# banyancomputer/hot-proofs-blake3-circom

Hardware: AMD Instinct MI355X
Metric: BLAKE3-compression witnesses/sec (higher is better)
Workload: dtype u32

## Files before the change

### hot-proofs-blake3-circom_amd/__init__.py

```python
import ctypes
import os
import re

import numpy as np

from . import workloads


def __getattr__(name):
    if name in ("sharding", "chain", "bao"):
        import importlib
        return importlib.import_module(__name__ + "." + name)
    raise AttributeError(name)

PKG_DIR = os.path.dirname(os.path.abspath(__file__))
LIB_PATH = os.environ.get("B3WIT_LIB") or os.path.join(PKG_DIR, "libb3wit.so")

CIRCUITS = ("compression", "nova_bn254", "nova_vesta", "nova_bn254_o1")
CIRCUIT_ID = {c: i for i, c in enumerate(CIRCUITS)}

B3W_OK = 0
PLACEMENT_NAMES = {0: "plain", 1: "mixed", 2: "interleaved"}
B3W_E_ASSERT_FAILED = 4
B3W_E_BAD_ARGUMENT = 100
# ... 65 lines not shown
        "b3w_bodies_stats": (i32, [vp, vp]),
        "b3w_bodies_search_stats": (i32, [vp, ctypes.POINTER(ctypes.c_double)]),
        "b3w_bodies_search_limit": (None, [ctypes.c_double]),
        "b3w_bodies_search_breakdown": (i32, [vp, ctypes.POINTER(ctypes.c_double)]),
        "b3w_bodies_store_rate": (i32, [vp, vp, u32, u64, i32, u32, vp, ctypes.POINTER(ctypes.c_double)]),
        "b3w_batch_placement": (i32, [vp]),
        "b3w_chain_num_chunks": (u64, [u64]),
        "b3w_chain_num_leaf_steps": (u64, [u64]),
        "b3w_chain_path_len": (u32, [u64, u64]),
        "b3w_chain_num_parent_steps": (u64, [u64, u64, u64]),
        "b3w_chain_parent_row": (u64, [u64, u64]),
        "b3w_chain_path_provable": (i32, [u64, u64]),
        "b3w_chain_plan_leaves_device": (i32, [vp, vp, u64, u64, u32, vp, vp, vp]),
        "b3w_chain_tree_device": (i32, [vp, vp, u64, vp, vp]),
        "b3w_chain_plan_parents_device": (i32, [vp, vp, u64, u64, u64, u32, vp, vp]),
        "b3w_commit_key_create": (i32, [vp, i32, u32, vp, ctypes.POINTER(vp)]),
        "b3w_commit_key_create_ex": (i32, [vp, i32, u32, vp, u32, ctypes.POINTER(vp)]),
        "b3w_commit_key_create_folded": (i32, [vp, i32, u32, vp, vp, u32, ctypes.POINTER(vp)]),
        "b3w_slot_widths": (i32, [vp, vp]),
        "b3w_commit_key_window": (u32, [vp]),
        "b3w_commit_key_destroy": (None, [vp]),
        "b3w_commit_key_count": (i32, [vp, i32]),
        "b3w_commit_key_counts": (i32, [vp, ctypes.POINTER(u64)]),
        "b3w_commit_records_device": (i32, [vp, vp, vp, u32, vp, vp, vp, vp]),
        "b3w_commit_records": (i32, [vp, vp, vp, u32, vp, vp, vp]),
        "b3w_chain_commit_only": (i32, [vp, vp, vp]),
        "b3w_chain_commit_from_records": (i32, [vp, vp, vp]),
        "b3w_chain_commit_overlap": (i32, [vp, i32]),
        "b3w_chain_violations_device": (vp, [vp]),
        "b3w_chain_commitments": (i32, [vp, vp, vp]),
        "b3w_chain_check_constraints": (i32, [vp, vp]),
        "b3w_chain_violations": (i32, [vp, vp, vp]),
        "b3w_batch_commit_device": (i32, [vp, vp, vp, u32, u64, vp, vp, vp]),
        "b3w_batch_commit": (i32, [vp, vp, vp, vp]),
        "b3w_commit_consumer": (None, [vp, vp, u64, u64, u32, vp]),
        "b3w_comm_unique_id": (i32, [vp]),
        "b3w_comm_create": (i32, [vp, vp, i32, i32, ctypes.POINTER(vp)]),
        "b3w_comm_create_host": (i32, [vp, ctypes.c_char_p, i32, i32, ctypes.POINTER(vp)]),
        "b3w_comm_create_external": (i32, [vp, i32, i32, vp, vp, ctypes.POINTER(vp)]),
        "b3w_comm_rank": (i32, [vp]),
        "b3w_comm_size": (i32, [vp]),
        "b3w_comm_destroy": (None, [vp]),
        "b3w_comm_allgather": (i32, [vp, vp, vp, u64, vp]),
        "b3w_batch_allgather_public": (i32, [vp, vp, vp]),
        "b3w_chain_create": (i32, [vp, u64, u64, u32, u32, u32, i32, ctypes.POINTER(vp)]),
        "b3w_chain_destroy": (None, [vp]),
# ... 40 lines not shown
        "b3w_bao_stream_outboard_begin": (i32, [vp, u64, u32, vp, vp, vp, u64, ctypes.POINTER(vp)]),
        "b3w_bao_stream_verify_begin": (i32, [vp, u64, u32, vp, vp, vp, vp, vp, vp, u64, vp, ctypes.POINTER(vp)]),
        "b3w_bao_stream_push": (i32, [vp, u64, vp, u64, vp]),
        "b3w_bao_stream_finish": (i32, [vp, vp]),
        "b3w_bao_stream_free": (None, [vp]),
        "b3w_sample_plan_arena_device": (i32, [vp, vp, u64, vp, vp, u32, u32, vp, vp, vp, vp, u32, vp, vp, vp]),
        "b3w_bao_slice_arena_device": (i32, [vp, vp, u64, vp, vp, u32, u32, vp, vp, vp, u32, vp, vp]),
    }
    for name, (res, args) in sig.items():
        fn = getattr(L, name)
        fn.restype, fn.argtypes = res, args
    _lib = L
    return L


EXPORTED_SYMBOLS = ("b3w_abi_version", "b3w_identify_wasm", "b3w_create", "b3w_destroy", "b3w_info",
                    "b3w_input_signal_size", "b3w_calc_witness", "b3w_write_wtns_header", "b3w_last_error",
                    "b3w_batch_run_device", "b3w_public_words", "b3w_batch_alloc", "b3w_batch_free",
                    "b3w_batch_run", "b3w_batch_outputs", "b3w_batch_fetch", "b3w_batch_device_ptr",
                    "b3w_batch_time_device", "b3w_batch_verify_device", "b3w_batch_verify",
                    "b3w_r1cs_create", "b3w_r1cs_info", "b3w_r1cs_is_tiled", "b3w_r1cs_destroy", "b3w_r1cs_check_device", "b3w_batch_r1cs_check", "b3w_r1cs_consumer", "b3w_batch_write_wtns", "b3w_batch_write_wtns_ex", "b3w_batch_autotune_device", "b3w_bodies_alloc", "b3w_bodies_free", "b3w_bodies_trim", "b3w_ctx_trim", "b3w_bodies_configure", "b3w_bodies_stats", "b3w_bodies_search_stats", "b3w_bodies_search_limit", "b3w_bodies_search_breakdown", "b3w_bodies_store_rate", "b3w_batch_placement", "b3w_chain_num_chunks", "b3w_chain_num_leaf_steps", "b3w_chain_path_len",
                    "b3w_chain_num_parent_steps", "b3w_chain_parent_row", "b3w_chain_path_provable",
                    "b3w_chain_plan_leaves_device", "b3w_chain_tree_device", "b3w_chain_plan_parents_device",
                    "b3w_commit_key_create", "b3w_commit_key_create_ex", "b3w_commit_key_create_folded", "b3w_slot_widths", "b3w_commit_key_window", "b3w_commit_key_destroy", "b3w_commit_key_count", "b3w_commit_key_counts", "b3w_commit_records_device", "b3w_commit_records", "b3w_chain_commit_only", "b3w_chain_commit_from_records", "b3w_chain_commit_overlap", "b3w_chain_violations_device", "b3w_chain_commitments", "b3w_chain_check_constraints", "b3w_chain_violations", "b3w_batch_commit_device", "b3w_batch_commit", "b3w_commit_consumer",
                    "b3w_comm_unique_id", "b3w_comm_create", "b3w_comm_create_host", "b3w_comm_create_external", "b3w_comm_rank", "b3w_comm_size", "b3w_comm_destroy", "b3w_comm_allgather", "b3w_batch_allgather_public",
                    "b3w_chain_create", "b3w_chain_destroy", "b3w_chain_run_leaves", "b3w_chain_run_parents", "b3w_chain_shard", "b3w_chain_run_parents_sharded", "b3w_chain_allgather_hout", "b3w_chain_allgather_hout_host", "b3w_chain_exchange_ms", "b3w_chain_info",
                    "b3w_chain_outputs", "b3w_chain_records", "b3w_chain_public", "b3w_chain_status", "b3w_chain_local_cvs", "b3w_chain_root",
                    "b3w_bao_outboard_size", "b3w_bao_outboard_device", "b3w_bao_path_nodes", "b3w_bao_slice", "b3w_sample_rows",
                    "b3w_sample_plan_device", "b3w_bao_batch_layout", "b3w_bao_batch_scratch_bytes", "b3w_bao_outboard_batch_device",
                    "b3w_sample_rows_batch", "b3w_sample_plan_batch_device", "b3w_bao_group_outboard_size", "b3w_bao_group_batch_layout",
                    "b3w_bao_group_path_nodes", "b3w_bao_group_outboard_batch_device", "b3w_sample_plan_group_batch_device",
                    "b3w_bao_slice_size", "b3w_bao_slice_batch_layout", "b3w_bao_slice_decode", "b3w_bao_slice_batch_device",
                    "b3w_sample_plan_slices_device",
                    "b3w_bao_verify_layout", "b3w_bao_verify_scratch_bytes", "b3w_bao_verify_batch_device", "b3w_bao_verify",
                    "b3w_bao_stream_scratch_bytes", "b3w_bao_stream_outboard_begin", "b3w_bao_stream_verify_begin", "b3w_bao_stream_push",
                    "b3w_bao_stream_finish", "b3w_bao_stream_free",
                    "b3w_sample_plan_arena_device", "b3w_bao_slice_arena_device")


class graph_capture:

    def __init__(self, graph, stream=None, **kw):
        import torch
        self._inner = torch.cuda.graph(graph, stream=stream, **kw)
        self._gc_was_on = False

    def __enter__(self):
# ... 346 lines not shown
    def commit_records_device(self, d_records, n, d_points, d_status, d_public=0, stream=0):
        rc = lib().b3w_commit_records_device(self.ctx.handle, self.handle, d_records, n, d_points, d_public or None, d_status, stream or None)
        if rc != B3W_OK:
            raise B3WError(rc, f"b3w_commit_records_device: status {rc}: {self.ctx.last_error()}")

    def commit_records(self, records):
        recs = np.ascontiguousarray(records, dtype=np.uint32)
        n = recs.shape[0]
        pts = np.zeros((n, 64), dtype=np.uint8)
        pub = np.zeros((n, self.ctx.public_words), dtype=np.uint32)
        st = np.zeros(n, dtype=np.int32)
        rc = lib().b3w_commit_records(self.ctx.handle, self.handle, recs.ctypes.data, n, pts.ctypes.data, pub.ctypes.data, st.ctypes.data)
        if rc != B3W_OK:
            raise B3WError(rc, f"b3w_commit_records: status {rc}: {self.ctx.last_error()}")
        return pts, pub, st

    def count(self, on=True):
        lib().b3w_commit_key_count(self.handle, 1 if on else 0)

    def counts(self):
        out = (ctypes.c_uint64 * 2)()
        lib().b3w_commit_key_counts(self.handle, out)
        return int(out[0]), int(out[1])

    def close(self):
        if getattr(self, "handle", None):
            lib().b3w_commit_key_destroy(self.handle)
            self.handle = None

    def __del__(self):
        try:
            self.close()
        except Exception:
            pass


class ChainPlanner:

    def __init__(self, ctx):
        self.ctx = ctx

    def _chk(self, rc, what):
        if rc != B3W_OK:
            raise B3WError(rc, f"{what}: status {rc}: {self.ctx.last_error()}")

    def parent_rows(self, n_chunks, first_chunk=0, n_chunks_local=None):
# ... 218 lines not shown
```

### hot-proofs-blake3-circom_amd/csrc/b3w_commit.hip

```cpp
#include <hip/hip_runtime.h>
#include <stdint.h>
#include <stdlib.h>
#include "b3w_kernels.h"
#include "b3w_atoms.h"

namespace {

struct Fp { uint32_t l[8]; };
struct Jac { Fp X, Y, Z; };

__device__ __forceinline__ bool fp_is_zero(const Fp &a) {
  uint32_t o = 0;
#pragma unroll
  for (int i = 0; i < 8; ++i) o |= a.l[i];
  return o == 0;
}
__device__ __forceinline__ bool fp_eq(const Fp &a, const Fp &b) {
  uint32_t o = 0;
#pragma unroll
  for (int i = 0; i < 8; ++i) o |= a.l[i] ^ b.l[i];
  return o == 0;
}
__device__ __forceinline__ Fp fp_zero() { Fp r; for (int i = 0; i < 8; ++i) r.l[i] = 0; return r; }

// ... 539 lines not shown
#pragma unroll
  for (int i = 0; i < 8; ++i) r2.l[i] = C.r2[i];
  const Fp gx = fp_mul(load_fp(gens + (uint64_t)s * 16), r2, C), gy = fp_mul(load_fp(gens + (uint64_t)s * 16 + 8), r2, C);
  const uint32_t *sc = inverses + 8ull * mag;
  Jac R = jac_infinity();
#pragma unroll 1
  for (int b = 255; b >= 0; --b) {
    R = jac_dbl(R, C);
    if ((sc[b >> 5] >> (b & 31)) & 1u) R = jac_madd(R, gx, gy, C);
  }
  Fp x, y, c32;
  jac_to_affine(R, x, y, C);
#pragma unroll
  for (int k = 0; k < 8; ++k) c32.l[k] = C.one[k];
#pragma unroll 1
  for (int k = 0; k < 5; ++k) c32 = fp_dbl(c32, C);
  const Fp xo = fp_mul(x, c32, C);
  store_fp(o, xo);
  store_fp(o + 8, fp_mul(y, c32, C));
  store_fp(on, xo);
  store_fp(on + 8, fp_mul(fp_sub(fp_zero(), y, C), c32, C));
}

#define B3W_WINDOW_K 4
template <int W>
__global__ __launch_bounds__(64) void b3w_commit_window_kernel(const uint32_t *__restrict__ points, uint32_t nwin,
                                                               uint32_t *__restrict__ table, B3wCurve C, B3wCurve9 C9) {
  constexpr int K = B3W_WINDOW_K;
  constexpr uint32_t CHUNKS = (1u << W) / K;
  __shared__ uint32_t lds[5 * K * 9 * 64];
  const uint32_t tid = threadIdx.x;
  const uint64_t gid = (uint64_t)blockIdx.x * 64 + tid;
  if (gid >= (uint64_t)nwin * CHUNKS) return;
  const uint32_t win = (uint32_t)(gid / CHUNKS), g0 = (uint32_t)(gid % CHUNKS) * K;
  auto at = [&](int what, int e, int l) -> uint32_t & { return lds[((what * K + e) * 9 + l) * 64 + tid]; };
  auto point = [&](uint32_t b, bool negate, F9 &x, F9 &y) {
    const uint32_t *pt = points + (uint64_t)(win * W + b) * 16;
    Fp py = load_fp(pt + 8);
    if (negate) py = fp_sub(fp_zero(), py, C);
    x = to29(load_fp(pt)); y = to29(py);
  };
  J9 acc = j9_infinity();
  const uint32_t m0 = g0 ^ (g0 >> 1);
#pragma unroll 1
  for (uint32_t b = 0; b < (uint32_t)W; ++b) {
    if (!((m0 >> b) & 1)) continue;
    F9 x, y;
    point(b, false, x, y);
    j9_madd(acc, x, y, C9);
  }
#pragma unroll 1
  for (int e = 0; e < K; ++e) {
    if (e > 0) {
      const uint32_t g = g0 + e, m = g ^ (g >> 1), b = (uint32_t)__builtin_ctz(g);
      F9 x, y;
      point(b, !((m >> b) & 1), x, y);
      j9_madd(acc, x, y, C9);
    }
    const F9 A = acc.inf ? one29(C9) : mul29(acc.ZZ, acc.ZZZ, C9);
#pragma unroll
    for (int l = 0; l < 9; ++l) {
      at(0, e, l) = acc.X.l[l]; at(1, e, l) = acc.Y.l[l];
      at(2, e, l) = acc.inf ? 0u : acc.ZZ.l[l]; at(3, e, l) = acc.inf ? 0u : acc.ZZZ.l[l];
    }
    F9 c;
    if (e == 0) c = A;
    else {
#pragma unroll
      for (int l = 0; l < 9; ++l) c.l[l] = at(4, e - 1, l);
      c = mul29(c, A, C9);
    }
#pragma unroll
    for (int l = 0; l < 9; ++l) at(4, e, l) = c.l[l];
  }
  F9 inv;
#pragma unroll
  for (int l = 0; l < 9; ++l) inv.l[l] = at(4, K - 1, l);
  inv = inv29(inv, C.pm2, C9);
#pragma unroll 1
  for (int e = K - 1; e >= 0; --e) {
// ... 351 lines not shown
  D.sp4[8] -= 1u;
  uint32_t x[8];
  for (int i = 0; i < 8; ++i) x[i] = C.one[i];
  for (int k = 0; k < 5; ++k) u256_dbl_mod_h(x, C.p);
  for (int i = 0; i < 8; ++i) w[i] = x[i];
  w[8] = 0;
  u288_split29(w, D.one);
  D.inv = C.inv & M29;
  const uint64_t phi = ((uint64_t)C.p[7] << 32) | C.p[6];
  D.mu = (uint32_t)((((unsigned __int128)1) << 77) / ((unsigned __int128)phi + 1));
  for (uint32_t k = 3; k <= 5; ++k) D.kp0[k - 3] = (k * D.p[0]) & M29;
  return D;
}

}

extern "C" int b3w_launch_commit_setup(const uint32_t *d_gens, const uint32_t *d_first_v, const uint32_t *d_nbits, uint32_t nslots,
                                       uint32_t *d_points, const B3wCurve *curve, hipStream_t stream) {
  if (!nslots) return 0;
  hipLaunchKernelGGL(b3w_commit_setup_kernel, dim3(nslots), dim3(64), 0, stream, d_gens, d_first_v, d_nbits, nslots, d_points, *curve);
  return (int)hipGetLastError();
}

extern "C" int b3w_launch_commit_windows(const uint32_t *d_points, uint32_t nwin, uint32_t window, uint32_t *d_table, const B3wCurve *curve, hipStream_t stream) {
  if (!nwin) return 0;
  if (!B3W_COMMIT_WINDOW_OK(window)) return (int)hipErrorInvalidValue;
  const uint64_t total = (uint64_t)nwin * ((1u << window) / B3W_WINDOW_K);
  const dim3 grid((uint32_t)((total + 63) / 64));
  const B3wCurve9 c9 = make_curve9(*curve);
  if (window == B3W_COMMIT_WINDOW_XL)
    hipLaunchKernelGGL(b3w_commit_window_kernel<B3W_COMMIT_WINDOW_XL>, grid, dim3(64), 0, stream, d_points, nwin, d_table, *curve, c9);
  else if (window == B3W_COMMIT_WINDOW_LARGE)
    hipLaunchKernelGGL(b3w_commit_window_kernel<B3W_COMMIT_WINDOW_LARGE>, grid, dim3(64), 0, stream, d_points, nwin, d_table, *curve, c9);
  else
    hipLaunchKernelGGL(b3w_commit_window_kernel<B3W_COMMIT_WINDOW_SMALL>, grid, dim3(64), 0, stream, d_points, nwin, d_table, *curve, c9);
  return (int)hipGetLastError();
}

extern "C" int b3w_launch_commit(const uint8_t *d_bodies, uint32_t n, uint64_t pitch, uint32_t first_slot, uint32_t nslots,
                                 const uint32_t *d_slotdesc, const uint32_t *d_images , uint32_t img_row, const uint32_t *d_runs,
                                 uint32_t nruns, const uint32_t *d_table, uint32_t nwin, uint32_t window,
                                 uint32_t *d_sums , uint8_t *d_out, int32_t *d_status,
                                 const uint32_t *d_invtab, uint32_t inv_nk, const uint32_t *d_invmeta, const uint32_t *d_aux,
                                 unsigned long long *d_adds, const B3wCurve *curve, hipStream_t stream) {
  if (!n) return 0;
  if (!d_images && !(d_invtab && d_invmeta && d_aux)) { d_invtab = nullptr; d_invmeta = nullptr; }
// ... 55 lines not shown
```

### hot-proofs-blake3-circom_amd/csrc/b3w_commit_api.cpp

```cpp
#include "b3w_internal.h"


struct b3w_commit_key {
  b3w_ctx *ctx = nullptr;
  B3wCurve curve{};
  uint32_t first_slot = 0, nwin = 0, window = 0;
  uint32_t nslots = 0;
  uint32_t *d_slotdesc = nullptr;
  uint32_t *d_runs = nullptr; uint32_t nruns = 0;
  uint32_t *d_images = nullptr; uint32_t images_cap = 0;
  uint32_t *d_table = nullptr;
  uint32_t *d_invtab = nullptr; uint32_t inv_nk = 0;
  uint32_t *d_invmeta = nullptr;
  uint32_t *d_sums = nullptr;
  uint32_t sums_cap = 0;
  unsigned long long *d_counts = nullptr;
  uint64_t host_witnesses = 0;
  bool counting = false;
};

namespace {
bool u256_geq(const uint32_t a[8], const uint32_t b[8]) { for (int i = 7; i >= 0; --i) if (a[i] != b[i]) return a[i] > b[i]; return true; }
void u256_sub_host(uint32_t a[8], const uint32_t b[8]) {
  uint64_t br = 0;
  for (int i = 0; i < 8; i++) { const uint64_t t = (uint64_t)a[i] - b[i] - br; a[i] = (uint32_t)t; br = (t >> 63) & 1; }
}
void u256_double_mod(uint32_t a[8], const uint32_t p[8]) {
  uint32_t c = 0;
  for (int i = 0; i < 8; i++) { const uint32_t n = (a[i] << 1) | c; c = a[i] >> 31; a[i] = n; }
  if (c || u256_geq(a, p)) u256_sub_host(a, p);
}
B3wCurve make_curve(const uint64_t p64[4]) {
  B3wCurve C{};
  memcpy(C.p, p64, 32);
  uint32_t x[8] = {1, 0, 0, 0, 0, 0, 0, 0};
  for (int i = 0; i < 256; i++) u256_double_mod(x, C.p);
  memcpy(C.one, x, 32);
  for (int i = 0; i < 256; i++) u256_double_mod(x, C.p);
  memcpy(C.r2, x, 32);
  memcpy(C.pm2, C.p, 32);
  const uint32_t two[8] = {2, 0, 0, 0, 0, 0, 0, 0};
  u256_sub_host(C.pm2, two);
  uint32_t inv = C.p[0];
  for (int i = 0; i < 5; i++) inv *= 2u - C.p[0] * inv;
  C.inv = 0u - inv;
  return C;
}
const uint64_t Q_BN254[4] = {0x3c208c16d87cfd47ull, 0x97816a916871ca8dull, 0xb85045b68181585dull, 0x30644e72e131a029ull};
const uint64_t P_VESTA_BASE[4] = {0x992d30ed00000001ull, 0x224698fc094cf91bull, 0x0ull, 0x4000000000000000ull};
}

extern "C" {

int32_t b3w_commit_key_create(b3w_ctx *ctx, int32_t curve, uint32_t first_slot, const uint8_t *host_generators, b3w_commit_key **out) {
  return b3w_commit_key_create_ex(ctx, curve, first_slot, host_generators, 0, out);
}

uint32_t b3w_commit_key_window(const b3w_commit_key *key) { return key ? key->window : 0; }

int32_t b3w_commit_key_create_ex(b3w_ctx *ctx, int32_t curve, uint32_t first_slot, const uint8_t *host_generators, uint32_t window_bits,
                                 b3w_commit_key **out) {
  return b3w_commit_key_create_folded(ctx, curve, first_slot, host_generators, nullptr, window_bits, out);
}

int32_t b3w_slot_widths(b3w_ctx *ctx, uint16_t *out_bits) {
  if (!ctx || !out_bits) return B3W_E_BAD_ARGUMENT;
  std::vector<uint32_t> table;
  if (!b3w_int_build_slot_table(ctx->desc, table, ctx->last_error)) return B3W_E_BAD_ARGUMENT;
  for (uint32_t i = 0; i < ctx->desc.nwit; i++) {
// ... 131 lines not shown
  if (e == hipSuccess) e = hipMalloc((void **)&key->d_slotdesc, (size_t)nslots * 4);
  if (e == hipSuccess) e = hipMemcpy(key->d_slotdesc, desc.data(), (size_t)nslots * 4, hipMemcpyHostToDevice);
  if (e == hipSuccess) e = hipMalloc((void **)&key->d_table, (size_t)key->nwin * B3W_COMMIT_ENTRIES(window) * 64);
  if (e == hipSuccess) e = hipMalloc((void **)&d_points, (size_t)nv * 64);
  if (e == hipSuccess) e = hipMalloc((void **)&d_gens, (size_t)nslots * 64);
  if (e == hipSuccess) e = hipMalloc((void **)&d_first, (size_t)nslots * 4);
  if (e == hipSuccess) e = hipMalloc((void **)&d_nbits, (size_t)nslots * 4);
  if (e == hipSuccess) e = hipMemcpy(d_gens, host_generators, (size_t)nslots * 64, hipMemcpyHostToDevice);
  if (e == hipSuccess) e = hipMemcpy(d_first, first_v.data(), (size_t)nslots * 4, hipMemcpyHostToDevice);
  if (e == hipSuccess) e = hipMemcpy(d_nbits, nbits.data(), (size_t)nslots * 4, hipMemcpyHostToDevice);
  int rc = e == hipSuccess ? b3w_launch_commit_setup(d_gens, d_first, d_nbits, nslots, d_points, &key->curve, nullptr) : 0;
  for (uint32_t v = V0; v < nv && e == hipSuccess && rc == 0; v++)
    e = hipMemcpyAsync(d_points + (size_t)v * 16, d_points, 64, hipMemcpyDeviceToDevice, nullptr);
  if (e == hipSuccess && rc == 0) rc = b3w_launch_commit_windows(d_points, key->nwin, key->window, key->d_table, &key->curve, nullptr);
  if (e == hipSuccess && rc == 0 && with_invtab) {
    key->inv_nk = B3W_INV_TABLE_N - 1;
    e = hipMalloc((void **)&key->d_invmeta, invmeta.size() * 4);
    if (e == hipSuccess) e = hipMemcpy(key->d_invmeta, invmeta.data(), invmeta.size() * 4, hipMemcpyHostToDevice);
    if (e == hipSuccess) e = hipMalloc((void **)&key->d_invtab, (size_t)B3W_NOVA_ISZERO * 2 * key->inv_nk * 64);
    if (e == hipSuccess)
      rc = b3w_launch_commit_invtab(d_gens, key->d_invmeta, static_cast<const uint32_t *>(ctx->d_aux) + 16, B3W_NOVA_ISZERO, key->inv_nk, key->d_invtab, &key->curve,
                                    nullptr);
  }
  if (e == hipSuccess && rc == 0) e = hipDeviceSynchronize();
  if (d_gens) (void)hipFree(d_gens);
  if (d_first) (void)hipFree(d_first);
  if (d_nbits) (void)hipFree(d_nbits);
  if (d_points) (void)hipFree(d_points);
  if (e != hipSuccess || rc != 0) {
    b3w_commit_key_destroy(key);
    *herr = e != hipSuccess ? e : (hipError_t)rc;
    (void)hipGetLastError();
    return hip_fail(ctx, e != hipSuccess ? e : (hipError_t)rc, "commitment key set-up");
  }
  *out = key;
  return B3W_OK;
}

void b3w_commit_key_destroy(b3w_commit_key *key) {
  if (!key) return;
  B3wCaptureRelaxed relaxed;
  DeviceGuard guard(key->ctx->device);
  if (key->d_slotdesc) (void)hipFree(key->d_slotdesc);
  if (key->d_invmeta) (void)hipFree(key->d_invmeta);
  if (key->d_runs) (void)hipFree(key->d_runs);
  if (key->d_images) (void)hipFree(key->d_images);
  if (key->d_table) (void)hipFree(key->d_table);
  if (key->d_invtab) (void)hipFree(key->d_invtab);
  if (key->d_sums) (void)hipFree(key->d_sums);
  if (key->d_counts) (void)hipFree(key->d_counts);
  delete key;
}

int32_t b3w_commit_key_count(b3w_commit_key *key, int32_t on) {
  if (!key) return B3W_E_BAD_ARGUMENT;
  b3w_ctx *ctx = key->ctx;
  ON_DEVICE(ctx);
  HIP_TRY(ctx, hipDeviceSynchronize());
  if (on && !key->d_counts) HIP_TRY(ctx, hipMalloc((void **)&key->d_counts, 8));
  if (on) { HIP_TRY(ctx, hipMemset(key->d_counts, 0, 8)); key->host_witnesses = 0; }
  key->counting = on != 0;
  return B3W_OK;
}

int32_t b3w_commit_key_counts(const b3w_commit_key *key, uint64_t out[2]) {
  if (!key || !out) return B3W_E_BAD_ARGUMENT;
  b3w_ctx *ctx = key->ctx;
  out[0] = 0; out[1] = key->host_witnesses;
  if (!key->d_counts) return B3W_OK;
  ON_DEVICE(ctx);
  HIP_TRY(ctx, hipDeviceSynchronize());
  unsigned long long v = 0;
  HIP_TRY(ctx, hipMemcpy(&v, key->d_counts, 8, hipMemcpyDeviceToHost));
  out[0] = v;
  return B3W_OK;
}

int32_t b3w_batch_commit_device(b3w_ctx *ctx, const b3w_commit_key *key, const uint8_t *d_bodies, uint32_t n, uint64_t pitch,
                                uint8_t *d_points, int32_t *d_status, void *stream) {
  if (!ctx || !key || key->ctx != ctx || !d_bodies || !d_points) return B3W_E_BAD_ARGUMENT;
  const uint64_t body = 32ull * ctx->desc.nwit;
  if (pitch == 0) pitch = body;
  if (pitch < body || (pitch & 15) || (reinterpret_cast<uintptr_t>(d_bodies) & 15) || (reinterpret_cast<uintptr_t>(d_points) & 15)) {
    ctx->last_error = "pitch must be >= witness_size*32 and a multiple of 16, bodies and points 16-byte aligned";
// ... 40 lines not shown
    return B3W_E_BAD_ARGUMENT;
  }
  ON_DEVICE(ctx);
  b3w_commit_key *k = const_cast<b3w_commit_key *>(key);
  constexpr uint32_t CHUNK = 32768;
  const uint32_t want = std::min(n, CHUNK);
  if (k->images_cap < want || k->sums_cap < want) {
    HIP_TRY(ctx, hipStreamSynchronize((hipStream_t)stream));
    if (split) HIP_TRY(ctx, hipStreamSynchronize((hipStream_t)trace_stream));
    if (k->sums_cap < want) {
      if (k->d_sums) (void)hipFree(k->d_sums);
      k->d_sums = nullptr; k->sums_cap = 0;
      HIP_TRY(ctx, hipMalloc((void **)&k->d_sums, (size_t)want * B3W_COMMIT_SUM_WORDS * 4));
      k->sums_cap = want;
    }
    if (k->images_cap < want) {
      if (k->d_images) (void)hipFree(k->d_images);
      k->d_images = nullptr; k->images_cap = 0;
      HIP_TRY(ctx, hipMalloc((void **)&k->d_images, (size_t)want * ctx->desc.lds_words * 4));
      k->images_cap = want;
    }
  }
  const uint32_t cap = k->images_cap;
  const uint32_t rw = ctx->desc.nin, pw = ctx->desc.npub;
  for (uint32_t c0 = 0; c0 < n; c0 += cap) {
    const uint32_t cn = std::min(cap, n - c0);
    int lrc = b3w_launch_trace(ctx->desc.kind, d_records + (uint64_t)c0 * rw, cn, k->d_images, cap, ctx->d_table, ctx->desc.nwit,
                               d_public ? d_public + (uint64_t)c0 * pw : nullptr, d_status + c0, ctx->d_aux, (hipStream_t)(split ? trace_stream : stream));
    if (lrc == 0 && split) {
      hipError_t e = hipEventRecord(trace_done, (hipStream_t)trace_stream);
      if (e == hipSuccess) e = hipStreamWaitEvent((hipStream_t)stream, trace_done, 0);
      if (e != hipSuccess) return hip_fail(ctx, e, "TRACE event");
    }
    if (lrc == 0)
      lrc = b3w_launch_commit(nullptr, cn, 0, key->first_slot, key->nslots, key->d_slotdesc, k->d_images, cap, key->d_runs, key->nruns,
                              key->d_table, key->nwin, key->window, d_sums_out ? d_sums_out + (uint64_t)c0 * B3W_COMMIT_SUM_WORDS : k->d_sums,
                              d_sums_out ? nullptr : d_points + (uint64_t)c0 * 64, nullptr, key->d_invtab, key->inv_nk,
                              nullptr, nullptr, key->counting ? key->d_counts : nullptr, &key->curve, (hipStream_t)stream);
    if (lrc == 0 && key->counting) k->host_witnesses += cn;
    if (lrc) return hip_fail(ctx, (hipError_t)lrc, "commit-from-records launch");
  }
  return B3W_OK;
}

extern "C" {

int32_t b3w_commit_records(b3w_ctx *ctx, const b3w_commit_key *key, const uint32_t *host_records, uint32_t n, uint8_t *host_points,
                           uint32_t *host_public, int32_t *host_status) {
  if (!ctx || !key || key->ctx != ctx || !host_records || !host_points) return B3W_E_BAD_ARGUMENT;
  if (n == 0) return B3W_OK;
  ON_DEVICE(ctx);
  const size_t rb = (size_t)n * ctx->desc.nin * 4, pb = (size_t)n * ctx->desc.npub * 4;
  uint8_t *d = nullptr;
  const size_t o_pts = (rb + 255) & ~(size_t)255, o_pub = o_pts + (size_t)n * 64, o_st = o_pub + ((pb + 255) & ~(size_t)255);
  HIP_TRY(ctx, hipMalloc((void **)&d, o_st + (size_t)n * 4));
  hipError_t e = hipMemset(d + o_pub, 0, o_st - o_pub);
  if (e == hipSuccess) e = hipMemcpy(d, host_records, rb, hipMemcpyHostToDevice);
  int32_t rc = B3W_OK;
  if (e == hipSuccess) rc = b3w_commit_records_device(ctx, key, reinterpret_cast<uint32_t *>(d), n, d + o_pts, reinterpret_cast<uint32_t *>(d + o_pub),
// ... 38 lines not shown
```

### hot-proofs-blake3-circom_amd/csrc/b3w_kernels.h

```cpp
#pragma once
#include <hip/hip_runtime_api.h>
#include <stdint.h>

#define B3W_VARIANT_SWEEP 100
#define B3W_VARIANT_SLICED 20
#define B3W_VARIANT_REGIONFILL 200
#define B3W_VARIANT_REGIONFILL_LIGHT 201
#define B3W_REGIONFILL_GRID 256
#define B3W_AUX_WIDE_SLOTS (16 + 8 * 2048)
#define B3W_AUX_LINE_COUNTS (B3W_AUX_WIDE_SLOTS + 68)
#define B3W_AUX_LINE_LISTS (B3W_AUX_LINE_COUNTS + 4)
#define B3W_LINE_LIST_MAX 160
#define B3W_AUX_ALIAS_COUNT (B3W_AUX_LINE_LISTS + 2 * 4 * B3W_LINE_LIST_MAX)
#define B3W_AUX_ALIAS_LIST (B3W_AUX_ALIAS_COUNT + 1)
#define B3W_ALIAS_MAX 192
#define B3W_SWEEP_GRID 256
#define B3W_SWEEP_LOGC 13
#define B3W_SWEEP_CHUNK (1u << B3W_SWEEP_LOGC)

extern "C" int b3w_launch_batch(int kind, int variant, const uint32_t *d_recs, uint32_t n, uint8_t *d_out,
                                uint64_t pitch, const uint32_t *d_table, uint32_t nwit, uint32_t *d_pub,
                                int32_t *d_status, const void *d_aux, uint32_t *d_scratch, uint32_t scratch_cap,
                                hipStream_t stream);

// ... 28 lines not shown
extern "C" void b3w_place_trim(void);
extern "C" void b3w_place_configure(int64_t search_gib, int64_t pool_gib);
extern "C" void b3w_place_stats(int device, uint64_t out[6]);
extern "C" void b3w_place_search_limit(double seconds);
extern "C" void b3w_place_search_stats(int device, double out[4]);
extern "C" void b3w_place_cost_breakdown(int device, double out[4]);
extern "C" int b3w_place_store_rate(uint8_t *buf, uint64_t pitch, uint32_t n, uint32_t body_bytes, int shape, uint32_t iters, hipStream_t stream, double *gbs);

#define B3W_COMMIT_WINDOW_SMALL 12
#define B3W_COMMIT_WINDOW_LARGE 16
#define B3W_COMMIT_WINDOW_XL 18
#define B3W_COMMIT_WINDOW_OK(w) ((w) == B3W_COMMIT_WINDOW_SMALL || (w) == B3W_COMMIT_WINDOW_LARGE || (w) == B3W_COMMIT_WINDOW_XL)
#define B3W_COMMIT_ENTRIES(W) ((1u << (W)) - 1u)
#define B3W_COMMIT_SUM_WORDS 36
struct B3wCurve {
  uint32_t p[8];
  uint32_t r2[8];
  uint32_t one[8];
  uint32_t pm2[8];
  uint32_t inv;
};
extern "C" int b3w_launch_commit_setup(const uint32_t *d_gens, const uint32_t *d_first_v, const uint32_t *d_nbits, uint32_t nslots,
                                       uint32_t *d_points, const B3wCurve *curve, hipStream_t stream);
extern "C" int b3w_launch_commit_windows(const uint32_t *d_points, uint32_t nwin, uint32_t window, uint32_t *d_table, const B3wCurve *curve, hipStream_t stream);
extern "C" int b3w_launch_commit(const uint8_t *d_bodies, uint32_t n, uint64_t pitch, uint32_t first_slot, uint32_t nslots,
                                 const uint32_t *d_slotdesc ,
                                 const uint32_t *d_images ,
                                 uint32_t img_row, const uint32_t *d_runs , uint32_t nruns,
                                 const uint32_t *d_table, uint32_t nwin, uint32_t window, uint32_t *d_sums, uint8_t *d_out,
                                 int32_t *d_status, const uint32_t *d_invtab , uint32_t inv_nk,
                                 const uint32_t *d_invmeta ,
                                 const uint32_t *d_aux ,
                                 unsigned long long *d_adds ,
                                 const B3wCurve *curve, hipStream_t stream);
extern "C" int b3w_launch_commit_normalize(const uint32_t *d_sums, uint64_t n, uint8_t *d_out, const B3wCurve *curve, hipStream_t stream);
#define B3W_NOVA_ISZERO 67
extern "C" int b3w_launch_commit_invtab(const uint32_t *d_gens, const uint32_t *d_inv_slot, const uint32_t *d_inverses, uint32_t njobs, uint32_t nk,
                                        uint32_t *d_invtab, const B3wCurve *curve, hipStream_t stream);

#include "b3w_r1cs_defs.h"
extern "C" int b3w_launch_r1cs(const uint8_t *d_bodies, uint32_t n, uint64_t pitch, uint32_t m, const uint32_t *d_rows,
                               const uint32_t *d_row_id, const uint32_t *d_wires, const uint16_t *d_cids, const uint32_t *d_coefR,
                               const B3wField *field, uint32_t *d_violations, uint32_t *d_first, hipStream_t stream);
struct B3wR1csSystem {
  uint32_t nwires, ntiles, max_ext, max_tile_terms, max_tile_rows, ncoef;
  const uint32_t *tiles, *tile_terms, *ext, *rows, *row_id, *row_k, *terms, *coefs;
// ... 30 lines not shown
```

### include/b3wit.h

```cpp
#ifndef B3WIT_H
#define B3WIT_H
#include <stddef.h>
#include <stdint.h>

#ifdef __cplusplus
extern "C" {
#endif

#define B3W_CIRCUIT_COMPRESSION_BN254 0
#define B3W_CIRCUIT_NOVA_BN254        1
#define B3W_CIRCUIT_NOVA_VESTA        2
#define B3W_CIRCUIT_NOVA_BN254_O1     3
#define B3W_CIRCUIT_UNKNOWN         (-1)

#define B3W_OK                     0
#define B3W_E_SIGNAL_NOT_FOUND     1
#define B3W_E_TOO_MANY_SIGNALS     2
#define B3W_E_SIGNAL_ALREADY_SET   3
#define B3W_E_ASSERT_FAILED        4
#define B3W_E_NOT_ENOUGH_MEMORY    5
#define B3W_E_ARRAY_ACCESS         6
#define B3W_E_BAD_ARGUMENT       100
#define B3W_E_NO_DEVICE          101
#define B3W_E_HIP                102
// ... 79 lines not shown
                                void *stream);

#define B3W_CURVE_BN254_G1 0
#define B3W_CURVE_PALLAS   1
#define B3W_CURVE_VESTA    B3W_CURVE_PALLAS
typedef struct b3w_commit_key b3w_commit_key;
int32_t b3w_commit_key_create(b3w_ctx *ctx, int32_t curve, uint32_t first_slot, const uint8_t *host_generators, b3w_commit_key **out);
int32_t b3w_commit_key_create_ex(b3w_ctx *ctx, int32_t curve, uint32_t first_slot, const uint8_t *host_generators, uint32_t window_bits,
                                 b3w_commit_key **out);
int32_t b3w_commit_key_create_folded(b3w_ctx *ctx, int32_t curve, uint32_t first_slot, const uint8_t *host_generators,
                                     const uint8_t *folded , uint32_t window_bits,
                                     b3w_commit_key **out);
int32_t b3w_slot_widths(b3w_ctx *ctx, uint16_t *out_bits );
uint32_t b3w_commit_key_window(const b3w_commit_key *key);
int32_t b3w_commit_key_count(b3w_commit_key *key, int32_t on);
int32_t b3w_commit_key_counts(const b3w_commit_key *key, uint64_t out[2]);
void b3w_commit_key_destroy(b3w_commit_key *key);
int32_t b3w_batch_commit_device(b3w_ctx *ctx, const b3w_commit_key *key, const uint8_t *d_bodies, uint32_t n, uint64_t pitch,
                                uint8_t *d_points , int32_t *d_status, void *stream);
int32_t b3w_batch_commit(b3w_batch *batch, const b3w_commit_key *key, uint8_t *host_points, int32_t *host_status);

int32_t b3w_commit_records_device(b3w_ctx *ctx, const b3w_commit_key *key, const uint32_t *d_records, uint32_t n, uint8_t *d_points,
                                  uint32_t *d_public, int32_t *d_status, void *stream);

int32_t b3w_commit_records(b3w_ctx *ctx, const b3w_commit_key *key, const uint32_t *host_records, uint32_t n, uint8_t *host_points,
                           uint32_t *host_public, int32_t *host_status);

typedef struct {
  b3w_ctx *ctx;
  const b3w_commit_key *key;
  uint8_t *d_points;
  int32_t *d_status;
  int32_t error;
} b3w_commit_sink;
void b3w_commit_consumer(void *user, const uint8_t *d_bodies, uint64_t pitch, uint64_t first_step, uint32_t count, void *stream);

int32_t b3w_batch_verify(b3w_batch *batch, uint32_t *host_mismatch);

int32_t b3w_batch_write_wtns(b3w_batch *batch, uint32_t first, uint32_t count, const char *dir, const char *prefix,
                             uint32_t *written);
int32_t b3w_batch_write_wtns_ex(b3w_batch *batch, uint32_t first, uint32_t count, const char *dir, const char *prefix,
                                uint32_t threads, uint32_t *written);

int32_t b3w_batch_autotune_device(b3w_ctx *ctx, const uint32_t *d_records, uint32_t n, uint8_t *d_bodies,
                                  uint64_t pitch, uint32_t *d_public, int32_t *d_status, void *stream,
                                  int32_t *chosen_variant, float *chosen_ms);
// ... 146 lines not shown
```

Baseline: 9.393 million.

## Merge commitment generators that read the same witness bit into one point

At key creation, a host-side plan groups all virtual generator slots that read the same source word/bit and sums their generator points on the device. A reduced set of window tables and runs is then built over these merged sources. The commit path uses the merged tables by default when they are available, which shrinks the number of windows and point additions per witness. This costs extra setup time and device memory, and adds a skip for zero (infinity) points in the window kernel.

```diff
diff --git a/hot-proofs-blake3-circom_amd/__init__.py b/hot-proofs-blake3-circom_amd/__init__.py
--- a/hot-proofs-blake3-circom_amd/__init__.py
+++ b/hot-proofs-blake3-circom_amd/__init__.py
@@ -111,6 +111,9 @@
         "b3w_commit_key_destroy": (None, [vp]),
         "b3w_commit_key_count": (i32, [vp, i32]),
         "b3w_commit_key_counts": (i32, [vp, ctypes.POINTER(u64)]),
+        "b3w_commit_key_merge": (i32, [vp, i32]),
+        "b3w_commit_key_merge_info": (i32, [vp, ctypes.POINTER(u32)]),
+        "b3w_commit_key_merge_plan": (i32, [vp, vp, vp, vp, u32]),
         "b3w_commit_records_device": (i32, [vp, vp, vp, u32, vp, vp, vp, vp]),
         "b3w_commit_records": (i32, [vp, vp, vp, u32, vp, vp, vp]),
         "b3w_chain_commit_only": (i32, [vp, vp, vp]),
@@ -197,7 +200,7 @@
                     "b3w_r1cs_create", "b3w_r1cs_info", "b3w_r1cs_is_tiled", "b3w_r1cs_destroy", "b3w_r1cs_check_device", "b3w_batch_r1cs_check", "b3w_r1cs_consumer", "b3w_batch_write_wtns", "b3w_batch_write_wtns_ex", "b3w_batch_autotune_device", "b3w_bodies_alloc", "b3w_bodies_free", "b3w_bodies_trim", "b3w_ctx_trim", "b3w_bodies_configure", "b3w_bodies_stats", "b3w_bodies_search_stats", "b3w_bodies_search_limit", "b3w_bodies_search_breakdown", "b3w_bodies_store_rate", "b3w_batch_placement", "b3w_chain_num_chunks", "b3w_chain_num_leaf_steps", "b3w_chain_path_len",
                     "b3w_chain_num_parent_steps", "b3w_chain_parent_row", "b3w_chain_path_provable",
                     "b3w_chain_plan_leaves_device", "b3w_chain_tree_device", "b3w_chain_plan_parents_device",
-                    "b3w_commit_key_create", "b3w_commit_key_create_ex", "b3w_commit_key_create_folded", "b3w_slot_widths", "b3w_commit_key_window", "b3w_commit_key_destroy", "b3w_commit_key_count", "b3w_commit_key_counts", "b3w_commit_records_device", "b3w_commit_records", "b3w_chain_commit_only", "b3w_chain_commit_from_records", "b3w_chain_commit_overlap", "b3w_chain_violations_device", "b3w_chain_commitments", "b3w_chain_check_constraints", "b3w_chain_violations", "b3w_batch_commit_device", "b3w_batch_commit", "b3w_commit_consumer",
+                    "b3w_commit_key_create", "b3w_commit_key_create_ex", "b3w_commit_key_create_folded", "b3w_slot_widths", "b3w_commit_key_window", "b3w_commit_key_destroy", "b3w_commit_key_count", "b3w_commit_key_counts", "b3w_commit_key_merge", "b3w_commit_key_merge_info", "b3w_commit_key_merge_plan", "b3w_commit_records_device", "b3w_commit_records", "b3w_chain_commit_only", "b3w_chain_commit_from_records", "b3w_chain_commit_overlap", "b3w_chain_violations_device", "b3w_chain_commitments", "b3w_chain_check_constraints", "b3w_chain_violations", "b3w_batch_commit_device", "b3w_batch_commit", "b3w_commit_consumer",
                     "b3w_comm_unique_id", "b3w_comm_create", "b3w_comm_create_host", "b3w_comm_create_external", "b3w_comm_rank", "b3w_comm_size", "b3w_comm_destroy", "b3w_comm_allgather", "b3w_batch_allgather_public",
                     "b3w_chain_create", "b3w_chain_destroy", "b3w_chain_run_leaves", "b3w_chain_run_parents", "b3w_chain_shard", "b3w_chain_run_parents_sharded", "b3w_chain_allgather_hout", "b3w_chain_allgather_hout_host", "b3w_chain_exchange_ms", "b3w_chain_info",
                     "b3w_chain_outputs", "b3w_chain_records", "b3w_chain_public", "b3w_chain_status", "b3w_chain_local_cvs", "b3w_chain_root",
@@ -590,6 +593,22 @@
         out = (ctypes.c_uint64 * 2)()
         lib().b3w_commit_key_counts(self.handle, out)
         return int(out[0]), int(out[1])
+
+    def merge(self, on=True):
+        return bool(lib().b3w_commit_key_merge(self.handle, 1 if on else 0))
+
+    def merge_info(self):
+        out = (ctypes.c_uint32 * 4)()
+        lib().b3w_commit_key_merge_info(self.handle, out)
+        return tuple(int(v) for v in out)
+
+    def merge_plan(self):
+        nv, ns, _, _ = self.merge_info()
+        src, off, mem = np.zeros(ns, dtype=np.uint32), np.zeros(ns + 1, dtype=np.uint32), np.zeros(max(nv, 1), dtype=np.uint32)
+        rc = lib().b3w_commit_key_merge_plan(self.handle, src.ctypes.data, off.ctypes.data, mem.ctypes.data, mem.size)
+        if rc != B3W_OK:
+            raise B3WError(rc, f"b3w_commit_key_merge_plan: status {rc}")
+        return src, off, mem[:int(off[-1])]
 
     def close(self):
         if getattr(self, "handle", None):
diff --git a/hot-proofs-blake3-circom_amd/csrc/b3w_commit.hip b/hot-proofs-blake3-circom_amd/csrc/b3w_commit.hip
--- a/hot-proofs-blake3-circom_amd/csrc/b3w_commit.hip
+++ b/hot-proofs-blake3-circom_amd/csrc/b3w_commit.hip
@@ -585,6 +585,30 @@
   store_fp(on + 8, fp_mul(fp_sub(fp_zero(), y, C), c32, C));
 }
 
+__global__ __launch_bounds__(64) void b3w_commit_merge_kernel(const uint32_t *__restrict__ points, const uint32_t *__restrict__ offsets,
+                                                              const uint32_t *__restrict__ members, uint32_t nsrc, uint32_t *__restrict__ merged,
+                                                              B3wCurve C, B3wCurve9 C9) {
+  const uint32_t s = blockIdx.x * 64 + threadIdx.x;
+  if (s >= nsrc) return;
+  J9 acc = j9_infinity();
+#pragma unroll 1
+  for (uint32_t i = offsets[s]; i < offsets[s + 1]; ++i) {
+    const uint32_t *pt = points + (uint64_t)members[i] * 16;
+    const Fp px = load_fp(pt), py = load_fp(pt + 8);
+    if (fp_is_zero(px) && fp_is_zero(py)) continue;
+    j9_madd(acc, to29(px), to29(py), C9);
+  }
+  Fp x = fp_zero(), y = fp_zero();
+  if (!acc.inf) {
+    const F9 ia = inv29(mul29(acc.ZZ, acc.ZZZ, C9), C.pm2, C9);
+    uint32_t hi;
+    x = from29(mul29(acc.X, mul29(ia, acc.ZZZ, C9), C9), hi); x = fp_reduce_once(x, hi, C);
+    y = from29(mul29(acc.Y, mul29(ia, acc.ZZ, C9), C9), hi); y = fp_reduce_once(y, hi, C);
+  }
+  store_fp(merged + (uint64_t)s * 16, x);
+  store_fp(merged + (uint64_t)s * 16 + 8, y);
+}
+
 #define B3W_WINDOW_K 4
 template <int W>
 __global__ __launch_bounds__(64) void b3w_commit_window_kernel(const uint32_t *__restrict__ points, uint32_t nwin,
@@ -599,9 +623,12 @@
   auto at = [&](int what, int e, int l) -> uint32_t & { return lds[((what * K + e) * 9 + l) * 64 + tid]; };
   auto point = [&](uint32_t b, bool negate, F9 &x, F9 &y) {
     const uint32_t *pt = points + (uint64_t)(win * W + b) * 16;
+    const Fp px = load_fp(pt);
     Fp py = load_fp(pt + 8);
+    if (fp_is_zero(px) && fp_is_zero(py)) return false;
     if (negate) py = fp_sub(fp_zero(), py, C);
-    x = to29(load_fp(pt)); y = to29(py);
+    x = to29(px); y = to29(py);
+    return true;
   };
   J9 acc = j9_infinity();
   const uint32_t m0 = g0 ^ (g0 >> 1);
@@ -609,16 +636,14 @@
   for (uint32_t b = 0; b < (uint32_t)W; ++b) {
     if (!((m0 >> b) & 1)) continue;
     F9 x, y;
-    point(b, false, x, y);
-    j9_madd(acc, x, y, C9);
+    if (point(b, false, x, y)) j9_madd(acc, x, y, C9);
   }
 #pragma unroll 1
   for (int e = 0; e < K; ++e) {
     if (e > 0) {
       const uint32_t g = g0 + e, m = g ^ (g >> 1), b = (uint32_t)__builtin_ctz(g);
       F9 x, y;
-      point(b, !((m >> b) & 1), x, y);
-      j9_madd(acc, x, y, C9);
+      if (point(b, !((m >> b) & 1), x, y)) j9_madd(acc, x, y, C9);
     }
     const F9 A = acc.inf ? one29(C9) : mul29(acc.ZZ, acc.ZZZ, C9);
 #pragma unroll
@@ -1016,6 +1041,14 @@
   return (int)hipGetLastError();
 }
 
+extern "C" int b3w_launch_commit_merge(const uint32_t *d_points, const uint32_t *d_offsets, const uint32_t *d_members, uint32_t nsrc,
+                                       uint32_t *d_merged, const B3wCurve *curve, hipStream_t stream) {
+  if (!nsrc) return 0;
+  hipLaunchKernelGGL(b3w_commit_merge_kernel, dim3((nsrc + 63) / 64), dim3(64), 0, stream, d_points, d_offsets, d_members, nsrc, d_merged, *curve,
+                     make_curve9(*curve));
+  return (int)hipGetLastError();
+}
+
 extern "C" int b3w_launch_commit_windows(const uint32_t *d_points, uint32_t nwin, uint32_t window, uint32_t *d_table, const B3wCurve *curve, hipStream_t stream) {
   if (!nwin) return 0;
   if (!B3W_COMMIT_WINDOW_OK(window)) return (int)hipErrorInvalidValue;
diff --git a/hot-proofs-blake3-circom_amd/csrc/b3w_commit_api.cpp b/hot-proofs-blake3-circom_amd/csrc/b3w_commit_api.cpp
--- a/hot-proofs-blake3-circom_amd/csrc/b3w_commit_api.cpp
+++ b/hot-proofs-blake3-circom_amd/csrc/b3w_commit_api.cpp
@@ -10,6 +10,11 @@
   uint32_t *d_runs = nullptr; uint32_t nruns = 0;
   uint32_t *d_images = nullptr; uint32_t images_cap = 0;
   uint32_t *d_table = nullptr;
+  uint32_t *d_table_m = nullptr; uint32_t nwin_m = 0;
+  uint32_t *d_runs_m = nullptr; uint32_t nruns_m = 0;
+  bool merge_on = true;
+  uint32_t nvirtual = 0;
+  std::vector<uint32_t> m_offsets, m_members, m_sources;
   uint32_t *d_invtab = nullptr; uint32_t inv_nk = 0;
   uint32_t *d_invmeta = nullptr;
   uint32_t *d_sums = nullptr;
@@ -45,6 +50,40 @@
   for (int i = 0; i < 5; i++) inv *= 2u - C.p[0] * inv;
   C.inv = 0u - inv;
   return C;
+}
+struct MergePlan { std::vector<uint32_t> offsets, members, sources, runs; };
+MergePlan merge_plan(const std::vector<uint32_t> &table, uint32_t first_slot, const uint8_t *folded, const std::vector<uint32_t> &nbits,
+                     const std::vector<uint32_t> &first_v) {
+  std::vector<std::pair<uint32_t, uint32_t>> reads;
+  for (uint32_t i = 0; i < (uint32_t)nbits.size(); i++) {
+    const uint32_t ent = table[first_slot + i], src = ent & 0xFFFu, sh = (ent >> 12) & 31u, v0 = first_v[i];
+    if (nbits[i] == 0) continue;
+    if (folded && (folded[i] & 0x80)) {
+      if (sh + (folded[i] & 31u) < 32) reads.emplace_back(src << 5 | (sh + (folded[i] & 31u)), v0);
+      continue;
+    }
+    for (uint32_t k = 0; k < nbits[i]; k++) {
+      const uint32_t word = k / 32, bit = ((word == 0 || word == 4) ? sh : 0u) + k % 32;
+      if (bit < 32) reads.emplace_back((src + word) << 5 | bit, v0 + k);
+    }
+  }
+  std::stable_sort(reads.begin(), reads.end(), [](const auto &a, const auto &b) { return a.first < b.first; });
+  MergePlan P;
+  for (size_t r = 0; r < reads.size(); r++) {
+    const uint32_t word = reads[r].first >> 5, bit = reads[r].first & 31u;
+    if (r == 0 || reads[r].first != reads[r - 1].first) {
+      const uint32_t s = (uint32_t)P.sources.size();
+      P.offsets.push_back((uint32_t)P.members.size());
+      P.sources.push_back(word | bit << 16);
+      const size_t nr = P.runs.size();
+      const uint32_t plen = nr ? (P.runs[nr - 2] >> 24) + 1 : 0;
+      if (nr && (P.runs[nr - 1] & 0xFFFFu) == word && (P.runs[nr - 1] >> 16) + plen == bit && plen < 32) P.runs[nr - 2] = (s - plen) | plen << 24;
+      else { P.runs.push_back(s | 0u << 24); P.runs.push_back(word | bit << 16); }
+    }
+    P.members.push_back(reads[r].second);
+  }
+  P.offsets.push_back((uint32_t)P.members.size());
+  return P;
 }
 const uint64_t Q_BN254[4] = {0x3c208c16d87cfd47ull, 0x97816a916871ca8dull, 0xb85045b68181585dull, 0x30644e72e131a029ull};
 const uint64_t P_VESTA_BASE[4] = {0x992d30ed00000001ull, 0x224698fc094cf91bull, 0x0ull, 0x4000000000000000ull};
@@ -222,6 +261,40 @@
       rc = b3w_launch_commit_invtab(d_gens, key->d_invmeta, static_cast<const uint32_t *>(ctx->d_aux) + 16, B3W_NOVA_ISZERO, key->inv_nk, key->d_invtab, &key->curve,
                                     nullptr);
   }
+  key->nvirtual = V0;
+  {
+    MergePlan plan = merge_plan(table, first_slot, folded, nbits, first_v);
+    key->m_offsets = std::move(plan.offsets); key->m_members = std::move(plan.members); key->m_sources = std::move(plan.sources);
+    const uint32_t nsrc = (uint32_t)key->m_sources.size(), nwin_m = (nsrc + window - 1) / window;
+    const uint64_t bytes_m = (uint64_t)nwin_m * B3W_COMMIT_ENTRIES(window) * 64;
+    size_t free_b = 0, total_b = 0;
+    if (e == hipSuccess && rc == 0 && nwin_m > 0 && nwin_m < key->nwin && hipMemGetInfo(&free_b, &total_b) == hipSuccess && bytes_m <= free_b / 4) {
+      uint32_t *d_off = nullptr, *d_mem = nullptr, *d_points_m = nullptr;
+      const size_t pts_m = (size_t)nwin_m * window * 64;
+      hipError_t me = hipMalloc((void **)&key->d_table_m, bytes_m);
+      if (me == hipSuccess) me = hipMalloc((void **)&d_points_m, pts_m);
+      if (me == hipSuccess) me = hipMemsetAsync(d_points_m, 0, pts_m, nullptr);
+      if (me == hipSuccess) me = hipMalloc((void **)&d_off, key->m_offsets.size() * 4);
+      if (me == hipSuccess) me = hipMemcpy(d_off, key->m_offsets.data(), key->m_offsets.size() * 4, hipMemcpyHostToDevice);
+      if (me == hipSuccess) me = hipMalloc((void **)&d_mem, key->m_members.size() * 4);
+      if (me == hipSuccess) me = hipMemcpy(d_mem, key->m_members.data(), key->m_members.size() * 4, hipMemcpyHostToDevice);
+      if (me == hipSuccess) me = hipMalloc((void **)&key->d_runs_m, plan.runs.size() * 4);
+      if (me == hipSuccess) me = hipMemcpy(key->d_runs_m, plan.runs.data(), plan.runs.size() * 4, hipMemcpyHostToDevice);
+      int mrc = me == hipSuccess ? b3w_launch_commit_merge(d_points, d_off, d_mem, nsrc, d_points_m, &key->curve, nullptr) : 0;
+      if (me == hipSuccess && mrc == 0) mrc = b3w_launch_commit_windows(d_points_m, nwin_m, window, key->d_table_m, &key->curve, nullptr);
+      if (me == hipSuccess && mrc == 0) me = hipDeviceSynchronize();
+      if (d_off) (void)hipFree(d_off);
+      if (d_mem) (void)hipFree(d_mem);
+      if (d_points_m) (void)hipFree(d_points_m);
+      if (me == hipSuccess && mrc == 0) { key->nwin_m = nwin_m; key->nruns_m = (uint32_t)(plan.runs.size() / 2); }
+      else if (me == hipErrorOutOfMemory) {
+        (void)hipGetLastError();
+        if (key->d_table_m) (void)hipFree(key->d_table_m);
+        if (key->d_runs_m) (void)hipFree(key->d_runs_m);
+        key->d_table_m = nullptr; key->d_runs_m = nullptr;
+      } else { e = me; rc = mrc; }
+    }
+  }
   if (e == hipSuccess && rc == 0) e = hipDeviceSynchronize();
   if (d_gens) (void)hipFree(d_gens);
   if (d_first) (void)hipFree(d_first);
@@ -246,6 +319,8 @@
   if (key->d_runs) (void)hipFree(key->d_runs);
   if (key->d_images) (void)hipFree(key->d_images);
   if (key->d_table) (void)hipFree(key->d_table);
+  if (key->d_table_m) (void)hipFree(key->d_table_m);
+  if (key->d_runs_m) (void)hipFree(key->d_runs_m);
   if (key->d_invtab) (void)hipFree(key->d_invtab);
   if (key->d_sums) (void)hipFree(key->d_sums);
   if (key->d_counts) (void)hipFree(key->d_counts);
@@ -260,6 +335,27 @@
   if (on && !key->d_counts) HIP_TRY(ctx, hipMalloc((void **)&key->d_counts, 8));
   if (on) { HIP_TRY(ctx, hipMemset(key->d_counts, 0, 8)); key->host_witnesses = 0; }
   key->counting = on != 0;
+  return B3W_OK;
+}
+
+int32_t b3w_commit_key_merge(b3w_commit_key *key, int32_t on) {
+  if (!key) return -1;
+  const int32_t was = key->merge_on ? 1 : 0;
+  key->merge_on = on != 0;
+  return was;
+}
+
+int32_t b3w_commit_key_merge_info(const b3w_commit_key *key, uint32_t out[4]) {
+  if (!key || !out) return B3W_E_BAD_ARGUMENT;
+  out[0] = key->nvirtual; out[1] = (uint32_t)key->m_sources.size(); out[2] = key->nwin; out[3] = key->nwin_m;
+  return B3W_OK;
+}
+
+int32_t b3w_commit_key_merge_plan(const b3w_commit_key *key, uint32_t *sources, uint32_t *offsets, uint32_t *members, uint32_t members_cap) {
+  if (!key || !sources || !offsets || !members || members_cap < key->m_members.size()) return B3W_E_BAD_ARGUMENT;
+  memcpy(sources, key->m_sources.data(), key->m_sources.size() * 4);
+  memcpy(offsets, key->m_offsets.data(), key->m_offsets.size() * 4);
+  memcpy(members, key->m_members.data(), key->m_members.size() * 4);
   return B3W_OK;
 }
 
@@ -346,6 +442,7 @@
     }
   }
   const uint32_t cap = k->images_cap;
+  const bool merged = key->merge_on && key->d_table_m && key->nwin_m;
   const uint32_t rw = ctx->desc.nin, pw = ctx->desc.npub;
   for (uint32_t c0 = 0; c0 < n; c0 += cap) {
     const uint32_t cn = std::min(cap, n - c0);
@@ -357,8 +454,8 @@
       if (e != hipSuccess) return hip_fail(ctx, e, "TRACE event");
     }
     if (lrc == 0)
-      lrc = b3w_launch_commit(nullptr, cn, 0, key->first_slot, key->nslots, key->d_slotdesc, k->d_images, cap, key->d_runs, key->nruns,
-                              key->d_table, key->nwin, key->window, d_sums_out ? d_sums_out + (uint64_t)c0 * B3W_COMMIT_SUM_WORDS : k->d_sums,
+      lrc = b3w_launch_commit(nullptr, cn, 0, key->first_slot, key->nslots, key->d_slotdesc, k->d_images, cap, merged ? key->d_runs_m : key->d_runs,
+                              merged ? key->nruns_m : key->nruns, merged ? key->d_table_m : key->d_table, merged ? key->nwin_m : key->nwin, key->window, d_sums_out ? d_sums_out + (uint64_t)c0 * B3W_COMMIT_SUM_WORDS : k->d_sums,
                               d_sums_out ? nullptr : d_points + (uint64_t)c0 * 64, nullptr, key->d_invtab, key->inv_nk,
                               nullptr, nullptr, key->counting ? key->d_counts : nullptr, &key->curve, (hipStream_t)stream);
     if (lrc == 0 && key->counting) k->host_witnesses += cn;
diff --git a/hot-proofs-blake3-circom_amd/csrc/b3w_kernels.h b/hot-proofs-blake3-circom_amd/csrc/b3w_kernels.h
--- a/hot-proofs-blake3-circom_amd/csrc/b3w_kernels.h
+++ b/hot-proofs-blake3-circom_amd/csrc/b3w_kernels.h
@@ -74,6 +74,8 @@
 };
 extern "C" int b3w_launch_commit_setup(const uint32_t *d_gens, const uint32_t *d_first_v, const uint32_t *d_nbits, uint32_t nslots,
                                        uint32_t *d_points, const B3wCurve *curve, hipStream_t stream);
+extern "C" int b3w_launch_commit_merge(const uint32_t *d_points, const uint32_t *d_offsets, const uint32_t *d_members, uint32_t nsrc,
+                                       uint32_t *d_merged, const B3wCurve *curve, hipStream_t stream);
 extern "C" int b3w_launch_commit_windows(const uint32_t *d_points, uint32_t nwin, uint32_t window, uint32_t *d_table, const B3wCurve *curve, hipStream_t stream);
 extern "C" int b3w_launch_commit(const uint8_t *d_bodies, uint32_t n, uint64_t pitch, uint32_t first_slot, uint32_t nslots,
                                  const uint32_t *d_slotdesc ,
diff --git a/include/b3wit.h b/include/b3wit.h
--- a/include/b3wit.h
+++ b/include/b3wit.h
@@ -125,6 +125,10 @@
 
 int32_t b3w_commit_records_device(b3w_ctx *ctx, const b3w_commit_key *key, const uint32_t *d_records, uint32_t n, uint8_t *d_points,
                                   uint32_t *d_public, int32_t *d_status, void *stream);
+
+int32_t b3w_commit_key_merge(b3w_commit_key *key, int32_t on);
+int32_t b3w_commit_key_merge_info(const b3w_commit_key *key, uint32_t out[4]);
+int32_t b3w_commit_key_merge_plan(const b3w_commit_key *key, uint32_t *sources, uint32_t *offsets, uint32_t *members, uint32_t members_cap);
 
 int32_t b3w_commit_records(b3w_ctx *ctx, const b3w_commit_key *key, const uint32_t *host_records, uint32_t n, uint8_t *host_points,
                            uint32_t *host_public, int32_t *host_status);
```

After: 9.399 million, median of 3. About the same (+0.1%).
